# LepistaBioinformatics/blutils

Hardware: AMD Instinct MI355X
Metric: Mqueries/sec consensus (synthetic outfmt-6 hit table) (higher is better)
Workload: dtype i32/u32

## Files before the change

blutils_amd/csrc/consensus_kernel.hip:

```cpp

#if defined(__HIP_DEVICE_COMPILE__) && !defined(__gfx950__)
#error "consensus_kernel.hip is written for gfx950"
#endif

#include <hip/hip_runtime.h>

#include <climits>
#include <cstdint>
#include <type_traits>

#include "blu_internal.h"

namespace blu {

#define WAVE 64

constexpr int BLOCK_A = 768;
constexpr int BLU_WAVES_PER_SIMD = 3;
constexpr int BLOCK_N = 1024;
constexpr int BLU_N_WAVES_PER_SIMD = 4;
constexpr int BLOCK_F = 704;
constexpr int LIST_CAP = 208;
constexpr int LIST_CAP_RING = 248;
constexpr int LIST_CAP_F64 = 232;
// ... 263 lines not shown
#define KEY_PID_BITS 17u
#define KEYED_LEN_SHIFT 25u
#define KEYED_PID_SHIFT 8u
#define PM_MASK ((1u << KEY_PID_BITS) - 1u)
#define LONG_SPAN (1u << 28)
#define KEEP_ROWS 1024u
#define SLOT_CAP 256u
#define TASK_SPAN (1ull << 27)
#define CUT_LDS 512
#define ROW_MASK ((1u << BLU_ROW_BITS) - 1u)
typedef uint32_t u32x2 __attribute__((ext_vector_type(2)));
typedef uint32_t u32x4 __attribute__((ext_vector_type(4)));

static_assert((RING_ROWS & RING_MASK) == 0 && RING_ROWS >= 1024u, "ring size");
#define DESC_SUB_BITS 8u
#define DESC_WORD1(RPL, row0, sub) (((row0) << DESC_SUB_BITS) | (sub))
static_assert(LIST_CAP >= 128 && LIST_CAP_RING >= 128 && LIST_CAP_F64 >= 128 && LIST_CAP_F64_RING >= 128, "the list area also stages the 64 records of a task");
static_assert(LIST_CAP_RING % 8 == 0 && LIST_CAP_RING <= 256 && LIST_CAP_F64_RING % 8 == 0 && LIST_CAP_F64_RING <= 256, "four list entries per lane in the gather");

struct FlatLds { uint32_t qs[WAVE + 4]; int32_t qm[WAVE]; uint32_t qk[WAVE]; };
struct NoFlatLds {};
template <bool F64, bool RING>
struct WaveLds : std::conditional_t<RING, NoFlatLds, FlatLds> {
    static constexpr uint32_t CAP = F64 ? (RING ? LIST_CAP_F64_RING : LIST_CAP_F64) : (RING ? LIST_CAP_RING : LIST_CAP);
    alignas(16) uint32_t ring[RING ? RING_ROWS + RING_PAD : 4u];
    uint4 rec[CAP];
    uint32_t p1[F64 ? CAP : 1];
    uint16_t pq[CAP];
    uint32_t meta[WAVE + 4];
    uint2 seg[WAVE + 4];
};

__device__ __forceinline__ void wait_vmcnt(uint32_t k) {
    switch (k) {
        case 0: asm volatile("s_waitcnt vmcnt(0)" ::: "memory"); break;
        case 1: asm volatile("s_waitcnt vmcnt(1)" ::: "memory"); break;
        case 2: asm volatile("s_waitcnt vmcnt(2)" ::: "memory"); break;
        case 3: asm volatile("s_waitcnt vmcnt(3)" ::: "memory"); break;
        case 4: asm volatile("s_waitcnt vmcnt(4)" ::: "memory"); break;
        case 5: asm volatile("s_waitcnt vmcnt(5)" ::: "memory"); break;
        case 6: asm volatile("s_waitcnt vmcnt(6)" ::: "memory"); break;
        case 7: asm volatile("s_waitcnt vmcnt(7)" ::: "memory"); break;
        case 8: asm volatile("s_waitcnt vmcnt(8)" ::: "memory"); break;
        case 9: asm volatile("s_waitcnt vmcnt(9)" ::: "memory"); break;
        case 10: asm volatile("s_waitcnt vmcnt(10)" ::: "memory"); break;
        case 11: asm volatile("s_waitcnt vmcnt(11)" ::: "memory"); break;
        case 12: asm volatile("s_waitcnt vmcnt(12)" ::: "memory"); break;
        case 13: asm volatile("s_waitcnt vmcnt(13)" ::: "memory"); break;
        case 14: asm volatile("s_waitcnt vmcnt(14)" ::: "memory"); break;
        default: asm volatile("s_waitcnt vmcnt(15)" ::: "memory"); break;
    }
}
static_assert(RING_CHUNKS <= 16, "wait_vmcnt covers 0..15 younger chunks");

template <int STRAT, int LAYOUT, bool RING>
__global__ __launch_bounds__((LAYOUT == 0 || LAYOUT == 3) ? (RING ? BLOCK_F : BLOCK_A) : (RING ? BLOCK_A : BLOCK_N), (RING || LAYOUT == 0 || LAYOUT == 3) ? BLU_WAVES_PER_SIMD : BLU_N_WAVES_PER_SIMD)
void blu_consensus_stream_kernel(HitsDev h, TaxDev t, blu_result* __restrict__ out, uint32_t* __restrict__ worklist, uint32_t* __restrict__ work_count,
                                 uint32_t mode, uint32_t* __restrict__ host_len) {
    const uint32_t forced = mode & 1u;
    const bool no_long = (mode & 2u) != 0u;
    constexpr bool PID32 = LAYOUT == 1 || LAYOUT == 2, PACKED = LAYOUT == 2, WIDE = LAYOUT == 3;
    constexpr uint32_t BLOCK_T = !PID32 ? (RING ? BLOCK_F : BLOCK_A) : (RING ? BLOCK_A : BLOCK_N), WAVES_T = BLOCK_T / WAVE;
    constexpr uint32_t CAP = WaveLds<!PID32, RING>::CAP;
    if (!forced && __hip_atomic_load(work_count + 9, __ATOMIC_RELAXED, __HIP_MEMORY_SCOPE_AGENT) != (RING ? 1u : 2u)) return;
    __shared__ WaveLds<!PID32, RING> s_lds[WAVES_T];
    constexpr bool CUT_TABLE = !PID32;
    __shared__ double s_cut[CUT_TABLE ? CUT_LDS : 1];
    const bool cut_in_lds = CUT_TABLE && t.n_cutvals <= CUT_LDS;
    if constexpr (CUT_TABLE) {
        if (cut_in_lds) {
            for (uint32_t i = threadIdx.x; i < t.n_cutvals; i += BLOCK_T) s_cut[i] = t.cutvals[i];
            __syncthreads();
        }
    }
    int lane = lane_id();
    const int wib = __builtin_amdgcn_readfirstlane(threadIdx.x / WAVE);
    WaveLds<!PID32, RING>& L = s_lds[wib];
    const uint32_t wl_cap = wl_capacity(h.n_queries);
    const uint32_t n_q32 = (uint32_t)h.n_queries;
    const uint32_t wave = blockIdx.x * WAVES_T + (uint32_t)wib;
    const uint32_t n_waves = gridDim.x * WAVES_T;
    uint32_t t_full, tail_q0, tail_nq;
    {
        const uint32_t n_tasks64 = n_q32 / WAVE + ((n_q32 % WAVE) != 0u ? 1u : 0u);
        t_full = n_tasks64 / n_waves * n_waves;
        const uint32_t q_full = t_full == n_tasks64 ? n_q32 : t_full * WAVE;
        uint32_t tail_q = (((n_q32 - q_full) + n_waves - 1u) / n_waves + 7u) / 8u * 8u;
        tail_q = tail_q < 16u ? 16u : (tail_q > WAVE ? WAVE : tail_q);
        const uint64_t p0 = (uint64_t)q_full + (uint64_t)wave * tail_q;
        tail_q0 = p0 < n_q32 ? (uint32_t)p0 : n_q32;
        tail_nq = n_q32 - tail_q0 < tail_q ? n_q32 - tail_q0 : tail_q;
    }

    const uint32_t mis = (uint32_t)(((uintptr_t)h.bitscore >> 2) & 3u);
    const char* const bs_al = reinterpret_cast<const char*>(h.bitscore) - 4u * mis;
    const uint64_t v_total = h.n_hits + mis;
    uint32_t ring_head = 0, ring_landed = 0, ring_tail = 0;
    uint32_t ring_c0 = 0, ring_end = 0;
    uint32_t pref_q0 = 0xFFFFFFFFu;
    u32x4 rs_ring = {0u, 0u, 0u, 0x00020000u};
    auto ring_desc = [&](const uint32_t c0) {
        const uint64_t left = (v_total - ((uint64_t)c0 << 8)) * 4ull;
        const uint64_t base = (uint64_t)(uintptr_t)bs_al + ((uint64_t)c0 << 10);
        return u32x4{(uint32_t)__builtin_amdgcn_readfirstlane((int)(uint32_t)base),
                     (uint32_t)__builtin_amdgcn_readfirstlane((int)((uint32_t)(base >> 32) & 0xFFFFu)),
                     (uint32_t)__builtin_amdgcn_readfirstlane((int)(left < 0x80000000ull ? (uint32_t)left : 0x80000000u)), 0x00020000u};
// ... 1 lines not shown
    const uint32_t ring_lds = (uint32_t)__builtin_amdgcn_readfirstlane((int)(uint32_t)(uintptr_t)(__attribute__((address_space(3))) void*)L.ring);
    auto ring_dma_run = [&](const u32x4 rs, const uint32_t c0, uint32_t head, const uint32_t lim) {
        uint32_t voff = (head - c0) * 1024u + (uint32_t)lane * 16u, keep, t;
        asm volatile("s_mov_b32 %[keep], m0\n"
                     "1:\n\t"
                     "s_and_b32 %[t], %[head], %[cm]\n\t"
                     "s_lshl_b32 %[t], %[t], 10\n\t"
                     "s_add_u32 m0, %[t], %[base]\n\t"
                     "s_add_u32 %[head], %[head], 1\n\t"
                     "buffer_load_dwordx4 %[voff], %[rs], 0 offen" RING_DMA_MOD " lds\n\t"
                     "v_add_u32 %[voff], 0x400, %[voff]\n\t"
                     "s_cmp_lt_u32 %[head], %[lim]\n\t"
                     "s_cbranch_scc1 1b\n\t"
                     "s_mov_b32 m0, %[keep]"
                     : [keep] "=&s"(keep), [t] "=&s"(t), [head] "+s"(head), [voff] "+v"(voff)
                     : [cm] "n"(RING_CHUNKS - 1u), [base] "s"(ring_lds), [rs] "s"(rs), [lim] "s"(lim) : "memory", "scc");
    };

    const uint32_t n_hits32 = (uint32_t)h.n_hits;
    auto load_seg = [&](const uint32_t tq0, const uint32_t tnq, uint32_t& o, uint32_t& e) {
        o = 0; e = 0;
        if ((uint32_t)lane < tnq) {
            const uint32_t* lo32 = reinterpret_cast<const uint32_t*>(h.seg_off + ((uint64_t)tq0 + (uint32_t)lane));
            o = lo32[0]; e = lo32[2];
        }
    };
    uint32_t nx_off, nx_end;
    uint32_t task = wave;
    bool in_tail = task >= t_full, tail_done = false;
    load_seg(in_tail ? tail_q0 : task * WAVE, in_tail ? tail_nq : (uint32_t)WAVE, nx_off, nx_end);

    for (; !in_tail || (tail_nq != 0u && !tail_done); tail_done = in_tail, task += n_waves, in_tail = task >= t_full) {
        __builtin_amdgcn_s_setprio(0);
        asm volatile("" : "+v"(lane));
        const uint32_t q0_32 = in_tail ? tail_q0 : task * WAVE;
        const uint64_t q0 = q0_32;
        const uint32_t nq = in_tail ? tail_nq : (uint32_t)WAVE;
        const uint32_t wl_sel = (uint32_t)(q0 / WAVE) & (WL_QUEUES - 1u);
        uint32_t* const wl_cnt = work_count + WL_BASE + wl_sel * WL_STRIDE;
        uint32_t* const wl_q = worklist + (uint64_t)wl_sel * wl_cap;
        uint32_t my_off = nx_off, my_end = nx_end;
        if (my_end > n_hits32) my_end = n_hits32;
        if (my_off > my_end) my_off = my_end;
        const bool nx_tail = task + n_waves >= t_full;
        const uint32_t nx_q0 = nx_tail ? tail_q0 : (task + n_waves) * WAVE;
        const uint32_t nx_nq = in_tail ? 0u : (nx_tail ? tail_nq : (uint32_t)WAVE);
        load_seg(nx_q0, nx_nq, nx_off, nx_end);
        asm volatile("" ::: "memory");
        uint32_t fill = 0;
        bool keyed = false;
        bool keyed_bad = false;
        uint32_t scan_rpl = 16;
        uint32_t fill_ring = 0;
        const uint64_t q = q0 + (uint32_t)lane;
        const uint32_t row0 = my_off;
        uint32_t mode = 3, r_len = 0, r_row = 0, r_pos = 0, r_hdr = 0, minlen = 0, d = 0, rec_kind = 0, g_lo = 0, g_hi = 0;
        typedef typename PidKey<PID32>::type PK;
        PK r_pid = 0, max_pid = 0;
        uint4 ra = {0, 0, 0, 0}, rb = {0, 0, 0, 0};
        uint32_t st_code = 0, st_ref = 0;
        uint32_t dn_flag = 0, dn_err = 0, dn_pos = 0, dn_k = 0;
        bool in_span = true;
        const uint32_t task_start = (uint32_t)rl((int)my_off, 0);
        const uint64_t rem = (uint64_t)(n_hits32 - task_start) < TASK_SPAN ? (uint64_t)(n_hits32 - task_start) : TASK_SPAN;
        const uint32_t rem4 = (uint32_t)(rem * 4), rem8 = (uint32_t)(rem * 8);
        const auto rs_bs = __builtin_amdgcn_make_buffer_rsrc((void*)(h.bitscore + task_start), 0, rem4, 0x00020000);
        const auto rs_tax = PACKED ? __builtin_amdgcn_make_buffer_rsrc((void*)(h.packed + 4ull * task_start), 0, (uint32_t)(rem * 16), 0x00020000)
                            : WIDE ? __builtin_amdgcn_make_buffer_rsrc((void*)(h.packed64 + 6ull * task_start), 0, (uint32_t)(rem * 24), 0x00020000)
                                   : __builtin_amdgcn_make_buffer_rsrc((void*)(h.tax_row + task_start), 0, rem4, 0x00020000);
        const auto rs_aln = __builtin_amdgcn_make_buffer_rsrc((void*)(h.align_len + task_start), 0, rem4, 0x00020000);
        const auto rs_acc = __builtin_amdgcn_make_buffer_rsrc((void*)(h.acc_rank + task_start), 0, rem4, 0x00020000);
        const auto rs_pid = (PACKED || WIDE) ? rs_tax : PID32 ? __builtin_amdgcn_make_buffer_rsrc((void*)(h.pident_milli + task_start), 0, rem4, 0x00020000)
                                  : __builtin_amdgcn_make_buffer_rsrc((void*)(h.pident + task_start), 0, rem8, 0x00020000);
        {
            const uint32_t nrows = my_end - my_off;
            in_span = my_off >= task_start && (my_end - task_start) <= (uint32_t)TASK_SPAN;
            L.seg[lane] = make_uint2(my_off - task_start, (nrows <= MAX_TASK_SEG && in_span) ? nrows : 0u);
        }
        const uint32_t task_rows = ((uint32_t)lane < nq ? my_end : 0u) - ((uint32_t)lane < nq ? task_start : 0u);
        bool contiguous, all_short;
        {
            const uint32_t rel_end = my_end - task_start, rel_off = my_off - task_start;
            const uint32_t prev_end = (uint32_t)__shfl_up((int)rel_end, 1);
            const bool ok = in_span && (lane == 0 || rel_off == prev_end);
            contiguous = __ballot((uint32_t)lane < nq && !ok) == 0ull;
            all_short = __ballot((uint32_t)lane < nq && (my_end - my_off) > SHORT_SEG) == 0ull;
        }
        const uint32_t task_nrows = (uint32_t)rl((int)task_rows, (int)nq - 1);
        const uint64_t vbase = (uint64_t)task_start + mis;
        const uint32_t seg_x = my_off - task_start;
        struct StepRegs { u32x4 vbs, vtax, vp01, vp23, valn, vacc, vq; int left; uint32_t qi; };
        auto fetch_rest = [&](StepRegs& R, const uint32_t voff, const uint32_t rows) {
            const bool any = voff != 0xFFFFFFF0u && rows != 0u;
            if (PACKED) {
                const uint32_t base = voff * 4u;
                R.vtax = __builtin_amdgcn_raw_buffer_load_b128(rs_tax, (any && (rows & 1u)) ? base : 0xFFFFFFC0u, 0, STREAM_AUX);
                R.vp01 = __builtin_amdgcn_raw_buffer_load_b128(rs_tax, (any && (rows & 2u)) ? base + 16u : 0xFFFFFFC0u, 0, STREAM_AUX);
                R.valn = __builtin_amdgcn_raw_buffer_load_b128(rs_tax, (any && (rows & 4u)) ? base + 32u : 0xFFFFFFC0u, 0, STREAM_AUX);
                R.vacc = __builtin_amdgcn_raw_buffer_load_b128(rs_tax, (any && (rows & 8u)) ? base + 48u : 0xFFFFFFC0u, 0, STREAM_AUX);
                R.vp23 = R.vp01;
                return;
            }
            if (WIDE) {
                const uint32_t base = voff * 6u;
                R.vtax = __builtin_amdgcn_raw_buffer_load_b128(rs_tax, (any && (rows & 1u)) ? base : 0xFFFFFFC0u, 0, STREAM_AUX);
                R.vp01 = __builtin_amdgcn_raw_buffer_load_b128(rs_tax, (any && (rows & 2u)) ? base + 24u : 0xFFFFFFC0u, 0, STREAM_AUX);
// ... 329 lines not shown
                if (st >= ns) break;
                const uint32_t q = um[st] & 63u, oq = (um[st] >> 6) & 63u;
                const bool have = ((um[st] >> 12) & 15u) != 0u;
                const int M = L.qm[q];
                const uint32_t tmask = (have && lmx[st] == M) ? (um[st] >> 16) & 0xFFu : 0u;
                const uint32_t c = (uint32_t)__builtin_popcount(tmask);
                uint32_t in2 = c;
                in2 += (uint32_t)dpp<0x111>((int)in2);
                in2 += (uint32_t)dpp<0x112>((int)in2);
                in2 += (uint32_t)dpp<0x114>((int)in2);
                in2 += (uint32_t)dpp<0x118>((int)in2);
                const uint32_t k0 = (uint32_t)rl((int)in2, 15), k1 = (uint32_t)rl((int)in2, 31), k2 = (uint32_t)rl((int)in2, 47), k3 = (uint32_t)rl((int)in2, 63);
                in2 += r16 == 0 ? 0u : (r16 == 1 ? k0 : (r16 == 2 ? k0 + k1 : k0 + k1 + k2));
                const uint32_t idx0 = running + in2 - c;
                if (have && oq == 0u) L.meta[q] = META_SLOW | idx0;
                if (c) atomicAdd(&L.qk[q], c);
                const bool over = have && idx0 + c > CAP;
                const uint64_t over_m = __ballot(over);
                const bool room = !over && c != 0u && (over_m == 0ull || (uint32_t)lane < (uint32_t)__builtin_ctzll(over_m));
                if (room) L.rec[idx0] = make_uint4(__builtin_bitreverse32(tmask), L.seg[q].x + UR * oq, UR * oq, 0u);
                if (over_m) { q_cut = (uint32_t)rl((int)q, __builtin_ctzll(over_m)); break; }
                running += k0 + k1 + k2 + k3;
            }
            __builtin_amdgcn_fence(__ATOMIC_RELEASE, "workgroup");
            __builtin_amdgcn_wave_barrier();
            __builtin_amdgcn_fence(__ATOMIC_ACQUIRE, "workgroup");
            const uint32_t m = L.meta[lane];
            if (rows != 0u && (uint32_t)lane < q_cut) L.meta[lane] = (m & 0xFFFFu) | (L.qk[lane] << 16);
            fill = q_cut < q_lim ? (L.meta[q_cut] & 0xFFFFu) : running;
            if (q_cut < WAVE) stop_q = q_cut;
            }
        };
        auto ring_mark_landed = [&](const uint32_t upto) {
            const uint32_t m0 = (ring_landed + RING_CHUNKS - 1u) & ~(RING_CHUNKS - 1u);
            if (m0 < upto) {
                if ((uint32_t)lane < RING_PAD) L.ring[RING_ROWS + lane] = L.ring[lane];
                __builtin_amdgcn_fence(__ATOMIC_RELEASE, "workgroup");
                __builtin_amdgcn_wave_barrier();
                __builtin_amdgcn_fence(__ATOMIC_ACQUIRE, "workgroup");
            }
            ring_landed = upto;
        };
        auto ring_refill = [&]() {
            if (ring_head < ring_tail) { ring_head = ring_tail; if (ring_landed < ring_tail) ring_landed = ring_tail; }
            const uint32_t lim = ring_end < ring_tail + RING_CHUNKS ? ring_end : ring_tail + RING_CHUNKS;
            if (ring_head < lim) { ring_dma_run(rs_ring, ring_c0, ring_head, lim); ring_head = lim; }
        };
        auto phase1_scan = [&](const auto rpl_c, const auto full_c, const uint32_t LPQ) {
            constexpr uint32_t RPL = decltype(rpl_c)::value;
            constexpr bool FULL = decltype(full_c)::value;
            static_assert(RPL <= RING_PAD && RPL <= 32u, "rows per lane");
            const uint32_t QPS = WAVE / LPQ;
            const uint32_t grp = (uint32_t)lane / LPQ, sub = ((uint32_t)lane & (LPQ - 1u)) * RPL, row16 = (uint32_t)lane >> 4;
            {
                const uint32_t cs = (uint32_t)((vbase + (uint32_t)rl((int)seg_x, (int)first_q)) >> 8);
                if (cs < ring_tail) { wait_vmcnt(0u); ring_head = ring_landed = ring_tail = cs; }
            }
            for (uint32_t qb = first_q / QPS * QPS; qb < nq; qb += QPS) {
                const uint32_t r_lo = (uint32_t)rl((int)seg_x, (int)(qb < first_q ? first_q : qb));
                const uint32_t qn = qb + QPS;
                const uint32_t r_hi = qn < nq ? (uint32_t)rl((int)seg_x, (int)qn) : task_nrows;
                ring_tail = (uint32_t)((vbase + r_lo) >> 8);
                ring_refill();
                if (r_hi > r_lo) {
                    const uint32_t need = (uint32_t)((vbase + r_hi - 1u) >> 8);
                    if (need >= ring_landed) { wait_vmcnt(ring_head - 1u - need); ring_mark_landed(need + 1u); }
                }
                const uint32_t qi = qb + grp;
                const uint2 sg = L.seg[qi];
                const int left0 = (sg.y > short_seg ? 0 : (int)sg.y) - (int)sub;
                const uint32_t over = (FULL && left0 > 0 && left0 < (int)RPL) ? RPL - (uint32_t)left0 : 0u;
                const uint32_t sub_e = sub - over;
                const int left = FULL ? (left0 > 0 ? (int)RPL : 0) : left0;
                const uint32_t row0 = sg.x + sub_e;
                const uint32_t a = ((uint32_t)vbase + sg.x + sub_e) & RING_MASK;
                int b[RPL];
#pragma unroll
                for (uint32_t i = 0; i < RPL; ++i) b[i] = (int)L.ring[a + i];
                asm volatile("s_waitcnt lgkmcnt(0)" ::: "memory");
#pragma unroll
                for (uint32_t i = 0; i < RPL; ++i) asm volatile("" : "+v"(b[i]));
                if (r_hi > r_lo) { ring_tail = (uint32_t)((vbase + r_hi) >> 8); ring_refill(); }
                int M = INT_MIN;
                if constexpr (FULL) {
#pragma unroll
                    for (uint32_t i = 0; i < RPL; ++i) M = imax(M, b[i]);
                    M = left > 0 ? M : INT_MIN;
                } else {
#pragma unroll
                    for (uint32_t i = 0; i < RPL; ++i) { b[i] = (int)i < left ? b[i] : INT_MIN; M = imax(M, b[i]); }
                }
                if (LPQ >= 2) M = imax(M, dpp<0xB1>(M));
                if (LPQ >= 4) M = imax(M, dpp<0x4E>(M));
                if (LPQ >= 8) M = imax(M, dpp<0x141>(M));
                if (LPQ >= 16) M = imax(M, dpp<0x140>(M));
                uint32_t mask = tie_mask<RPL>(b, M);
                mask = left > 0 ? mask : 0u;
                if constexpr (FULL) mask &= 0xFFFFFFFFu >> (32u - RPL + over);
                const uint32_t c = (uint32_t)__builtin_popcount(mask);
                uint32_t incl = c;
                incl += (uint32_t)dpp<0x111>((int)incl);
                incl += (uint32_t)dpp<0x112>((int)incl);
                incl += (uint32_t)dpp<0x114>((int)incl);
                incl += (uint32_t)dpp<0x118>((int)incl);
                const uint32_t k0 = (uint32_t)rl((int)incl, 15), k1 = (uint32_t)rl((int)incl, 31);
                const uint32_t k2 = (uint32_t)rl((int)incl, 47), k3 = (uint32_t)rl((int)incl, 63);
                const bool fits = fill + k0 + k1 + k2 + k3 <= CAP;
                const uint32_t p1 = fill + k0, p2 = p1 + k1, p3 = p2 + k2;
                const uint32_t rbase = row16 == 0 ? fill : (row16 == 1 ? p1 : (row16 == 2 ? p2 : p3));
                uint32_t gk = c;
                if (LPQ >= 2) gk += (uint32_t)dpp<0xB1>((int)gk);
                if (LPQ >= 4) gk += (uint32_t)dpp<0x4E>((int)gk);
                if (LPQ >= 8) gk += (uint32_t)dpp<0x141>((int)gk);
                if (LPQ >= 16) gk += (uint32_t)dpp<0x140>((int)gk);
                if (PID32 && !fits) {
                    __builtin_amdgcn_s_setprio(2);
                    uint64_t BK = 0;
                    uint32_t bacc = 0, bpos = 0, brow = 0, kmin = 0xFFFFFFFFu, pmax = 0, dlo = 0xFFFFFFFFu, dhi = 0, err = 0xFFFFFFFFu;
                    auto reset = [&]() { BK = 0; bacc = 0; bpos = 0; brow = 0; kmin = 0xFFFFFFFFu; pmax = 0; dlo = 0xFFFFFFFFu; dhi = 0; err = 0xFFFFFFFFu; };
                    auto better = [&](const uint64_t K, const uint32_t acc, const uint32_t pos, const uint64_t K2, const uint32_t acc2, const uint32_t pos2) {
                        const bool gt = (K > K2) | ((K == K2) & (acc > acc2)), eq = (K == K2) & (acc == acc2);
                        return STRAT == BLU_RELAXED ? (gt | (eq & (pos > pos2))) : ((!gt & !eq) | (eq & (pos < pos2)));
                    };
                    auto take_record = [&](const u32x4 rec, const uint32_t gp, const bool on) {
                        const uint32_t len = umin(rec.x >> BLU_ROW_BITS, t.max_depth), pos = rec.x & ROW_MASK;
                        const bool unmatched = pos >= t.n_tax, bad = !unmatched && (rec.x >> BLU_ROW_BITS) == 0;
                        const uint32_t e = (gp << 8) | (bad ? (uint32_t)BLU_ST_ERR_BAD_LINEAGE : (uint32_t)BLU_ST_ERR_UNMATCHED_TAXID);
                        err = (on && (unmatched | bad)) ? umin(err, e) : err;
                        const uint32_t pm = rec.y & ((1u << KEY_PID_BITS) - 1u);
                        const uint32_t k1 = (len << KEY_PID_BITS) | pm;
                        const uint64_t K = ((uint64_t)k1 << 32) | (rec.z ^ 0x80000000u);
                        const bool take = on & ((kmin == 0xFFFFFFFFu) | better(K, rec.w, gp, BK, bacc, bpos));
                        BK = take ? K : BK; bacc = take ? rec.w : bacc; bpos = take ? gp : bpos; brow = take ? pos : brow;
                        kmin = on ? umin(kmin, k1) : kmin;
                        const uint32_t pmo = pm | ((!PACKED && rec.y >= (1u << KEY_PID_BITS)) ? 0x80000000u : 0u);
                        pmax = (on && pmo > pmax) ? pmo : pmax;
                        dlo = on ? umin(dlo, pos) : dlo;
                        dhi = (on && pos > dhi) ? pos : dhi;
                    };
                    auto load_record = [&](const uint32_t row, const bool on) {
                        u32x4 r;
                        if (PACKED) r = __builtin_amdgcn_raw_buffer_load_b128(rs_tax, on ? row * 16u : 0xFFFFFFC0u, 0, GATHER_AUX);
                        else {
                            const uint32_t o4 = on ? row * 4u : 0xFFFFFFF0u;
                            r.x = __builtin_amdgcn_raw_buffer_load_b32(rs_tax, o4, 0, GATHER_AUX);
                            r.y = __builtin_amdgcn_raw_buffer_load_b32(rs_pid, o4, 0, GATHER_AUX);
                            r.z = __builtin_amdgcn_raw_buffer_load_b32(rs_aln, o4, 0, GATHER_AUX);
                            r.w = __builtin_amdgcn_raw_buffer_load_b32(rs_acc, o4, 0, GATHER_AUX);
                        }
                        return r;
                    };
                    auto merge = [&](auto ctrl) {
                        constexpr int C = decltype(ctrl)::value;
                        const uint64_t K2 = ((uint64_t)(uint32_t)dpp<C>((int)(uint32_t)(BK >> 32)) << 32) | (uint32_t)dpp<C>((int)(uint32_t)BK);
                        const uint32_t acc2 = (uint32_t)dpp<C>((int)bacc), pos2 = (uint32_t)dpp<C>((int)bpos), row2 = (uint32_t)dpp<C>((int)brow);
                        const uint32_t kmin2 = (uint32_t)dpp<C>((int)kmin);
                        const bool take = (kmin2 != 0xFFFFFFFFu) & ((kmin == 0xFFFFFFFFu) | better(K2, acc2, pos2, BK, bacc, bpos));
                        BK = take ? K2 : BK; bacc = take ? acc2 : bacc; bpos = take ? pos2 : bpos; brow = take ? row2 : brow;
                        kmin = umin(kmin, kmin2);
                        const uint32_t pm2 = (uint32_t)dpp<C>((int)pmax); pmax = pm2 > pmax ? pm2 : pmax;
                        dlo = umin(dlo, (uint32_t)dpp<C>((int)dlo));
                        const uint32_t hi2 = (uint32_t)dpp<C>((int)dhi); dhi = hi2 > dhi ? hi2 : dhi;
                        err = umin(err, (uint32_t)dpp<C>((int)err));
                    };
                    auto deliver = [&](const int src, const bool mine) {
                        const uint32_t f_khi = (uint32_t)__builtin_amdgcn_ds_bpermute(src, (int)(uint32_t)(BK >> 32));
                        const uint32_t f_pos = (uint32_t)__builtin_amdgcn_ds_bpermute(src, (int)bpos), f_row = (uint32_t)__builtin_amdgcn_ds_bpermute(src, (int)brow);
// ... 43 lines not shown
                            if (LPQ >= 2) merge(std::integral_constant<int, 0x141>());
                            if (LPQ >= 4) merge(std::integral_constant<int, 0x140>());
                            deliver((int)(((own0 & 15u) * 4u) * 4u), mine && (own0 >> 4) == g);
                        }
                    } else {
                        uint32_t m = mask;
                        while (__ballot(m != 0u)) {
                            u32x4 rq[4];
                            uint32_t gp[4];
#pragma unroll
                            for (int j = 0; j < 4; ++j) {
                                const bool on = m != 0u;
                                const uint32_t hb = on ? 31u - (uint32_t)__builtin_clz(m) : 0u, i = RPL - 1u - hb;
                                m = on ? (m & ~(1u << hb)) : 0u;
                                gp[j] = on ? sub_e + i : 0xFFFFFFFFu;
                                rq[j] = load_record(row0 + i, on);
                            }
#pragma unroll
                            for (int j = 0; j < 4; ++j) take_record(rq[j], gp[j], gp[j] != 0xFFFFFFFFu);
                        }
                        if (LPQ >= 2) merge(std::integral_constant<int, 0xB1>());
                        if (LPQ >= 4) merge(std::integral_constant<int, 0x4E>());
                        if (LPQ >= 8) merge(std::integral_constant<int, 0x141>());
                        if (LPQ >= 16) merge(std::integral_constant<int, 0x140>());
                        deliver((int)(own0 * 4u), mine);
                    }
                    {
                        const uint32_t f_gk = (uint32_t)__builtin_amdgcn_ds_bpermute((int)(own0 * 4u), (int)gk);
                        dn_k = (mine && dn_flag == 1u) ? f_gk : dn_k;
                    }
                    if (sub == 0 && gk != 0u) L.meta[qi] = META_DENSE;
                    __builtin_amdgcn_s_setprio(0);
                    continue;
                }
                uint32_t idx = rbase + incl - c;
                if (!fits) {
                    const uint32_t lane_o = (uint32_t)__builtin_ctzll(__ballot(idx + c > CAP));
                    const uint32_t qo = qb + lane_o / LPQ;
                    const bool taken = qi < qo;
                    if (sub == 0) L.meta[qi] = taken ? (idx | (gk << 16)) : META_SLOW;
                    if (taken && c) { L.rec[idx].x = mask << (32u - RPL); L.rec[idx].y = DESC_WORD1(RPL, row0, sub_e); }
                    fill = (uint32_t)rl((int)idx, (int)((qo - qb) * LPQ));
                    stop_q = qo;
                    wait_vmcnt(0u);
                    ring_head = ring_landed = ring_tail = (uint32_t)((vbase + (uint32_t)rl((int)seg_x, (int)qo)) >> 8);
                    break;
                }
                if (sub == 0) L.meta[qi] = idx | (gk << 16);
                fill = p3 + k3;
                static_assert((RPL == 16u || RPL == 32u) && SHORT_SEG <= 128u, "descriptor word of a lane");
                if (c) { L.rec[idx].x = mask << (32u - RPL); L.rec[idx].y = DESC_WORD1(RPL, row0, sub_e); }
            }
        };
        auto gather_list = [&](auto&& between) {
            constexpr int NG = (CAP + WAVE - 1) / WAVE;
            u32x4 g[NG];
            uint32_t ghi[NG], gpos[NG], ghint[NG];
            uint32_t carry = 0;
#pragma unroll
            for (int u = 0; u < NG; ++u) {
                g[u] = u32x4{0u, 0u, 0u, 0u}; ghi[u] = 0u; gpos[u] = 0u; ghint[u] = 0u;
                if ((uint32_t)u * WAVE >= fill_ring) continue;
                const uint32_t idx = (uint32_t)u * WAVE + (uint32_t)lane;
                const bool valid = idx < fill_ring;
                const uint32_t d0 = L.rec[idx < CAP ? idx : 0u].x;
                int s = (valid && d0 != 0u) ? (int)idx : 0;
                s = imax(s, dpp<0x111>(s));
                s = imax(s, dpp<0x112>(s));
                s = imax(s, dpp<0x114>(s));
                s = imax(s, dpp<0x118>(s));
                s = imax(s, __builtin_amdgcn_update_dpp(0, s, 0x142, 0xA, 0xF, false));
                s = imax(s, __builtin_amdgcn_update_dpp(0, s, 0x143, 0xC, 0xF, false));
                s = imax(s, (int)carry);
                carry = (uint32_t)rl(s, 63);
                const uint4 dd = L.rec[s];
                const uint32_t d0w = dd.x, d = dd.y;
                uint32_t r = idx - (uint32_t)s, x = scan_rpl == 32u ? d0w : d0w >> 16, i = 0;
                if (scan_rpl == 32u) {
                    const uint32_t h = x >> 16, ch = (uint32_t)__builtin_popcount(h);
                    const bool low = r >= ch;
                    r -= low ? ch : 0u; x = low ? (x & 0xFFFFu) : h; i += low ? 16u : 0u;
                }
                {
                    const uint32_t h = x >> 8, ch = (uint32_t)__builtin_popcount(h);
                    const bool low = r >= ch;
                    r -= low ? ch : 0u; x = low ? (x & 0xFFu) : h; i += low ? 8u : 0u;
                }
                {
                    const uint32_t h = x >> 4, ch = (uint32_t)__builtin_popcount(h);
                    const bool low = r >= ch;
                    r -= low ? ch : 0u; x = low ? (x & 0xFu) : h; i += low ? 4u : 0u;
                }
                {
                    const uint32_t h = x >> 2, ch = (uint32_t)__builtin_popcount(h);
                    const bool low = r >= ch;
                    r -= low ? ch : 0u; x = low ? (x & 0x3u) : h; i += low ? 2u : 0u;
                }
                i += (r >= (x >> 1)) ? 1u : 0u;
                const uint32_t row = (RING ? (d >> DESC_SUB_BITS) : d) + i;
                gpos[u] = (RING ? (d & ((1u << DESC_SUB_BITS) - 1u)) : dd.z) + i;
                if (PACKED) g[u] = __builtin_amdgcn_raw_buffer_load_b128(rs_tax, valid ? row * 16u : 0xFFFFFFC0u, 0, GATHER_AUX);
                else if (WIDE) {
                    g[u] = __builtin_amdgcn_raw_buffer_load_b128(rs_tax, valid ? row * 24u : 0xFFFFFFC0u, 0, GATHER_AUX);
                    const u32x2 p = __builtin_amdgcn_raw_buffer_load_b64(rs_tax, valid ? row * 24u + 16u : 0xFFFFFFE0u, 0, GATHER_AUX);
                    ghint[u] = g[u].y;
                    g[u].y = p.x; ghi[u] = p.y;
                } else {
                    const uint32_t o4 = valid ? row * 4u : 0xFFFFFFF0u;
                    g[u].x = __builtin_amdgcn_raw_buffer_load_b32(rs_tax, o4, 0, GATHER_AUX);
                    if (PID32) g[u].y = __builtin_amdgcn_raw_buffer_load_b32(rs_pid, o4, 0, GATHER_AUX);
                    else {
                        const u32x2 p = __builtin_amdgcn_raw_buffer_load_b64(rs_pid, valid ? row * 8u : 0xFFFFFFE0u, 0, GATHER_AUX);
                        g[u].y = p.x; ghi[u] = p.y;
                    }
                    g[u].z = __builtin_amdgcn_raw_buffer_load_b32(rs_aln, o4, 0, GATHER_AUX);
                    g[u].w = __builtin_amdgcn_raw_buffer_load_b32(rs_acc, o4, 0, GATHER_AUX);
                }
            }
            between();
            bool ovf = false;
            uint32_t gk[NG];
#pragma unroll
            for (int u = 0; u < NG; ++u) {
                const bool valid = (uint32_t)u * WAVE + (uint32_t)lane < fill_ring;
                if constexpr (PID32) { gk[u] = g[u].y & PM_MASK; ovf |= !PACKED && valid && g[u].y >= (1u << KEY_PID_BITS); }
                else {
                    const double p = __hiloint2double((int)ghi[u], (int)g[u].y);
                    const bool in_range = p >= 0.0 && p < 131.0705;
                    const uint32_t k = in_range ? (uint32_t)(p * 1000.0 + 0.5) : 0u;
                    const double back = milli17_to_f64(k);
                    gk[u] = k;
                    ovf |= valid && !(in_range && __double2hiint(back) == (int)ghi[u] && __double2loint(back) == (int)g[u].y && k < BLU_KTHR_NEVER);
                }
            }
            keyed = __ballot(ovf) == 0ull && fill == fill_ring;
            bool any_bad = false;
#pragma unroll
            for (int u = 0; u < NG; ++u) {
                const uint32_t idx = (uint32_t)u * WAVE + (uint32_t)lane;
                if (idx < fill_ring) {
                    if (keyed) {
                        const uint32_t len = umin(g[u].x >> BLU_ROW_BITS, t.max_depth);
                        any_bad |= len == 0u || (g[u].x & ROW_MASK) >= t.n_tax;
                        const uint32_t hint = (PID32 ? g[u].y : ghint[u]) >> KEY_PID_BITS;
                        L.rec[idx] = make_uint4((g[u].x & ROW_MASK) | ((hint >> 8) << BLU_ROW_BITS),
                                                (len << KEYED_LEN_SHIFT) | (gk[u] << KEYED_PID_SHIFT) | (hint & 0xFFu), g[u].z ^ 0x80000000u, g[u].w);
                    } else L.rec[idx] = make_uint4(g[u].x, g[u].y, g[u].z, g[u].w);
                    L.pq[idx] = (uint16_t)gpos[u];
                    if (!PID32) L.p1[idx] = ghi[u];
                }
            }
            keyed_bad = __ballot(any_bad) != 0ull;
        };
        bool pend = (uint32_t)lane < nq;
        uint32_t pend_before = WAVE + 1;
        if (RING && contiguous) {
            ring_c0 = (uint32_t)(vbase >> 8);
            rs_ring = ring_desc(ring_c0);
            ring_end = task_nrows ? (uint32_t)((vbase + task_nrows - 1u) >> 8) + 1u : ring_c0;
            if (pref_q0 != q0_32) ring_head = ring_landed = ring_c0;
            ring_tail = ring_c0;
        }
        for (;;) {
        fill = 0;
        stop_q = WAVE;
        bool ring_round = false;
        bool list_round = false;
        keyed = false;
        {
            const uint32_t rows = L.seg[lane].y;
            const uint64_t live = __ballot(rows != 0u);
            first_q = live ? (uint32_t)__builtin_ctzll(live) : 0u;
            {
                const uint32_t n16 = (uint32_t)__builtin_popcountll(__ballot(rows != 0u && rows <= 16u));
                const uint32_t n32 = (uint32_t)__builtin_popcountll(__ballot(rows != 0u && rows <= 32u));
                const uint32_t n64 = (uint32_t)__builtin_popcountll(__ballot(rows != 0u && rows <= 64u));
                const uint32_t n128 = (uint32_t)__builtin_popcountll(__ballot(rows != 0u && rows <= SHORT_SEG));
                const uint32_t c16 = 4u * n16 + BLU_LONG_COST * (n128 - n16), c32 = 8u * n32 + BLU_LONG_COST * (n128 - n32);
                const uint32_t c64 = 16u * n64 + BLU_LONG_COST * (n128 - n64), c128 = 32u * n128;
                uint32_t best = c128;
                short_seg = SHORT_SEG;
                if (c64 < best) { best = c64; short_seg = 64u; }
                if (c32 < best) { best = c32; short_seg = 32u; }
                if (c16 < best) { best = c16; short_seg = 16u; }
            }
            bool flat_round = false;
            if constexpr (!RING) {
                const uint32_t n128 = (uint32_t)__builtin_popcountll(__ballot(rows != 0u && rows <= SHORT_SEG));
                const uint32_t n_over = (uint32_t)__builtin_popcountll(__ballot(rows > SHORT_SEG));
                uint32_t best;
                {
                    const uint32_t n16 = (uint32_t)__builtin_popcountll(__ballot(rows != 0u && rows <= 16u));
                    const uint32_t n32 = (uint32_t)__builtin_popcountll(__ballot(rows != 0u && rows <= 32u));
                    const uint32_t n64 = (uint32_t)__builtin_popcountll(__ballot(rows != 0u && rows <= 64u));
                    best = 32u * n128;
                    best = umin(best, 16u * n64 + BLU_LONG_COST * (n128 - n64));
                    best = umin(best, 8u * n32 + BLU_LONG_COST * (n128 - n32));
                    best = umin(best, 4u * n16 + BLU_LONG_COST * (n128 - n16));
                }
                const uint32_t units = (uint32_t)wave_sum_u32((rows + FLAT_ROWS - 1u) / FLAT_ROWS);
                flat_round = units != 0u && units + units / 4u + 64u < best + BLU_LONG_COST * n_over;
                if (flat_round) { short_seg = FLAT_SEG; scan_rpl = 16u; }
            }
            const uint32_t longest = flat_round ? 0u : wave_max_u32(rows > short_seg ? 0u : rows);
            ring_round = RING && contiguous && longest != 0u && all_short && __ballot(rows > short_seg) == 0ull;
            uint32_t lpq = 1;
            if (ring_round) {
                scan_rpl = longest > 32u ? 32u : 16u;
                while (lpq * scan_rpl < longest) lpq *= 2;
                while ((WAVE / lpq) * longest + 256u > RING_ROWS) lpq *= 2;
            }
            list_round = ring_round || flat_round;
            if (list_round) {
#pragma unroll
                for (uint32_t u = 0; u * WAVE < CAP; ++u) { const uint32_t i = u * WAVE + (uint32_t)lane; if (i < CAP) L.rec[i].x = 0u; }
            }
            if (ring_round) {
                const bool all_full = __ballot(rows != 0u && rows <= short_seg && rows < scan_rpl) == 0ull;
                if (scan_rpl == 32u) {
                    if (all_full) phase1_scan(std::integral_constant<uint32_t, 32>(), std::true_type(), lpq);
                    else phase1_scan(std::integral_constant<uint32_t, 32>(), std::false_type(), lpq);
                } else phase1_scan(std::integral_constant<uint32_t, 16>(), std::false_type(), lpq);
            }
            else if (flat_round) phase1_flat();
            else if (longest > 32u && longest <= 64u) phase1(std::integral_constant<uint32_t, 16>(), false);
            else if (longest) phase1(longest <= 16u ? 4u : (longest <= 32u ? 8u : 32u), longest >= (PACKED ? 9u : 25u));
            if (stop_q < WAVE && rows != 0u && ((uint32_t)lane >= stop_q || rows > short_seg)) L.meta[lane] = META_SLOW;
            fill_ring = list_round ? fill : 0u;
            const uint64_t long_mask = __ballot(rows > short_seg);
            if (long_mask && stop_q == WAVE) phase1_long(long_mask);
        }
        __builtin_amdgcn_fence(__ATOMIC_RELEASE, "workgroup");
        __builtin_amdgcn_wave_barrier();
        __builtin_amdgcn_fence(__ATOMIC_ACQUIRE, "workgroup");
        const bool last_round = __ballot(pend && (my_end - my_off) != 0u && (my_end - my_off) <= MAX_TASK_SEG && in_span && (L.meta[lane] & META_SLOW)) == 0ull;
        uint32_t nxt_c0 = 0, nxt_lim = 0;
        if (RING && last_round && nx_nq != 0u) {
            uint32_t n_off = nx_off, n_end = nx_end;
            asm volatile("" : "+v"(n_off), "+v"(n_end));
            if (n_end > n_hits32) n_end = n_hits32;
            if (n_off > n_end) n_off = n_end;
            const uint32_t nqn = nx_nq;
            const uint32_t n_start = (uint32_t)rl((int)n_off, 0);
            const bool n_span = n_off >= n_start && (n_end - n_start) <= (uint32_t)TASK_SPAN;
            const uint32_t rel_end = n_end - n_start, rel_off = n_off - n_start;
            const uint32_t prev_end = (uint32_t)__shfl_up((int)rel_end, 1);
            const bool ok = n_span && (n_end - n_off) <= SHORT_SEG && (lane == 0 || rel_off == prev_end);
            const uint32_t n_rows = (uint32_t)rl((int)rel_end, (int)nqn - 1);
            if (__ballot((uint32_t)lane < nqn && !ok) == 0ull && n_rows != 0u) {
                const uint64_t vb = (uint64_t)n_start + mis;
                nxt_c0 = (uint32_t)(vb >> 8);
                const uint32_t cend = (uint32_t)((vb + n_rows - 1u) >> 8) + 1u;
                nxt_lim = cend < nxt_c0 + RING_CHUNKS ? cend : nxt_c0 + RING_CHUNKS;
            }
        }
        auto prefetch_next = [&]() {
            if (nxt_lim > nxt_c0) {
                const auto rsn = ring_desc(nxt_c0);
                ring_dma_run(rsn, nxt_c0, nxt_c0, nxt_lim);
                ring_head = nxt_lim; ring_landed = nxt_c0; ring_tail = nxt_c0;
                pref_q0 = nx_q0;
            }
        };
        __builtin_amdgcn_s_setprio(3);
        if (list_round) gather_list(prefetch_next);
        else prefetch_next();
        __builtin_amdgcn_fence(__ATOMIC_RELEASE, "workgroup");
        __builtin_amdgcn_wave_barrier();
        __builtin_amdgcn_fence(__ATOMIC_ACQUIRE, "workgroup");

        {
            const uint32_t nrows = my_end - my_off;
            const uint32_t m = L.meta[lane];
            const bool listed = pend && nrows != 0 && nrows <= MAX_TASK_SEG && in_span && !(m & (META_SLOW | META_DENSE));
            const uint32_t first = listed ? (m & 0xFFFFu) : 0u, k = listed ? ((m >> 16) & 0x3FFu) : 0u;
            const uint32_t kmax = wave_max_u32(k);
            uint32_t err = 0, err_pos = 0, nan_pos = 0xFFFFFFFFu;
            uint32_t b_len = 0, b_acc = 0, lo = 0xFFFFFFFFu, hi = 0, l_minlen = 0xFFFFFFFFu, l_row = 0, l_pos = 0, l_hint = 0;
            int b_aln = 0;
            PK b_pid = 0, l_maxpid = 0;
            const uint32_t last_e = k ? k - 1u : 0u;
            uint4 nx_rec = make_uint4(0, 0, 0, 0);
            uint32_t nx_pq = 0;
            uint32_t l_keyed = 0;
            if (!keyed) { nx_rec = L.rec[first]; nx_pq = L.pq[first]; }
            if (keyed) {
                l_keyed = 1u;
                uint64_t BK = 0;
                uint32_t kmin = 0xFFFFFFFFu, pmax = 0;
                uint32_t l_idx = first;
                auto step = [&](const auto check_c, const uint4 x, const uint32_t xidx, const bool is_first) {
                    const uint32_t pos = x.x & ROW_MASK;
                    if constexpr (decltype(check_c)::value) {
                        const bool unmatched = pos >= t.n_tax, bad = x.y < (1u << KEYED_LEN_SHIFT);
                        const bool first_err = (err == 0) & (unmatched | bad);
                        err = first_err ? (unmatched ? (uint32_t)BLU_ST_ERR_UNMATCHED_TAXID : (uint32_t)BLU_ST_ERR_BAD_LINEAGE) : err;
                        err_pos = first_err ? (uint32_t)L.pq[xidx] : err_pos;
                    }
                    kmin = umin(kmin, x.y);
                    lo = umin(lo, pos);
                    hi = pos > hi ? pos : hi;
                    const uint32_t ky = x.y & ~0xFFu;
                    const uint32_t pm = (x.y >> KEYED_PID_SHIFT) & PM_MASK;
                    pmax = pm > pmax ? pm : pmax;
                    const uint64_t K = ((uint64_t)ky << 32) | x.z;
                    const bool gt = (K > BK) | ((K == BK) & (x.w > b_acc)), eq = (K == BK) & (x.w == b_acc);
                    const bool take = is_first | (STRAT == BLU_RELAXED ? (gt | eq) : !(gt | eq));
                    BK = take ? K : BK;
                    b_acc = take ? x.w : b_acc;
                    l_idx = take ? xidx : l_idx;
                };
                auto reduce = [&](const auto check_c) {
                    for (uint32_t e = 0; e < kmax; e += 4) {
                        uint4 x[4];
                        uint32_t xi[4];
// ... 728 lines not shown
```

Before: 11400.

## Gather packed taxonomy rows via direct-to-LDS DMA and defer overflowing scan groups

For the packed ring layout, the list gather now issues buffer_load ... lds instructions that write the gathered 16-byte taxonomy records straight into LDS behind the ring. The wait is counted, so the next task's ring prefetch can stay in flight while the gather completes, and the results are then re-keyed in place. When a scan group would overflow the list, the scan stops early, saves that group's descriptor, and resumes it in a later round instead of taking the slow fallback path. This avoids register staging and the full vmcnt drain, at the cost of inline asm with manual m0 juggling and more complex round state.

```diff
diff --git a/blutils_amd/csrc/consensus_kernel.hip b/blutils_amd/csrc/consensus_kernel.hip
--- a/blutils_amd/csrc/consensus_kernel.hip
+++ b/blutils_amd/csrc/consensus_kernel.hip
@@ -339,6 +339,9 @@
     }
 }
 static_assert(RING_CHUNKS <= 16, "wait_vmcnt covers 0..15 younger chunks");
+constexpr uint32_t GATHER_REQS = (LIST_CAP_RING + WAVE - 1) / WAVE;
+static_assert(RING_CHUNKS + GATHER_REQS <= 15u, "ring chunks and gather requests in flight together fit the counted wait");
+__device__ __forceinline__ void gather_wait(const uint32_t chunks_behind) { wait_vmcnt(chunks_behind); }
 
 template <int STRAT, int LAYOUT, bool RING>
 __global__ __launch_bounds__((LAYOUT == 0 || LAYOUT == 3) ? (RING ? BLOCK_F : BLOCK_A) : (RING ? BLOCK_A : BLOCK_N), (RING || LAYOUT == 0 || LAYOUT == 3) ? BLU_WAVES_PER_SIMD : BLU_N_WAVES_PER_SIMD)
@@ -446,6 +449,8 @@
         bool keyed_bad = false;
         uint32_t scan_rpl = 16;
         uint32_t fill_ring = 0;
+        uint32_t dz_mask = 0, dz_w1 = 0, dz_qb = 0, dz_lpq = 0, scan_from = 0xFFFFFFFFu;
+        bool dz_on = false;
         const uint64_t q = q0 + (uint32_t)lane;
         const uint32_t row0 = my_off;
         uint32_t mode = 3, r_len = 0, r_row = 0, r_pos = 0, r_hdr = 0, minlen = 0, d = 0, rec_kind = 0, g_lo = 0, g_hi = 0;
@@ -881,11 +886,12 @@
             static_assert(RPL <= RING_PAD && RPL <= 32u, "rows per lane");
             const uint32_t QPS = WAVE / LPQ;
             const uint32_t grp = (uint32_t)lane / LPQ, sub = ((uint32_t)lane & (LPQ - 1u)) * RPL, row16 = (uint32_t)lane >> 4;
-            {
+            const bool resume = PACKED && scan_from != 0xFFFFFFFFu;
+            if (!resume) {
                 const uint32_t cs = (uint32_t)((vbase + (uint32_t)rl((int)seg_x, (int)first_q)) >> 8);
                 if (cs < ring_tail) { wait_vmcnt(0u); ring_head = ring_landed = ring_tail = cs; }
             }
-            for (uint32_t qb = first_q / QPS * QPS; qb < nq; qb += QPS) {
+            for (uint32_t qb = resume ? scan_from : first_q / QPS * QPS; qb < nq; qb += QPS) {
                 const uint32_t r_lo = (uint32_t)rl((int)seg_x, (int)(qb < first_q ? first_q : qb));
                 const uint32_t qn = qb + QPS;
                 const uint32_t r_hi = qn < nq ? (uint32_t)rl((int)seg_x, (int)qn) : task_nrows;
@@ -942,6 +948,11 @@
                 if (LPQ >= 4) gk += (uint32_t)dpp<0x4E>((int)gk);
                 if (LPQ >= 8) gk += (uint32_t)dpp<0x141>((int)gk);
                 if (LPQ >= 16) gk += (uint32_t)dpp<0x140>((int)gk);
+                if (PACKED && !fits && fill != 0u && k0 + k1 + k2 + k3 <= CAP) {
+                    dz_mask = mask << (32u - RPL); dz_w1 = DESC_WORD1(RPL, row0, sub_e); dz_qb = qb; dz_lpq = LPQ; dz_on = true;
+                    stop_q = qb;
+                    break;
+                }
                 if (PID32 && !fits) {
                     __builtin_amdgcn_s_setprio(2);
                     uint64_t BK = 0;
@@ -1091,8 +1102,104 @@
                 if (c) { L.rec[idx].x = mask << (32u - RPL); L.rec[idx].y = DESC_WORD1(RPL, row0, sub_e); }
             }
         };
+        auto entry_of = [&](const uint32_t idx, const bool valid, uint32_t& carry, uint32_t& row, uint32_t& pos) {
+            const uint32_t d0 = L.rec[idx < CAP ? idx : 0u].x;
+            int s = (valid && d0 != 0u) ? (int)idx : 0;
+            s = imax(s, dpp<0x111>(s));
+            s = imax(s, dpp<0x112>(s));
+            s = imax(s, dpp<0x114>(s));
+            s = imax(s, dpp<0x118>(s));
+            s = imax(s, __builtin_amdgcn_update_dpp(0, s, 0x142, 0xA, 0xF, false));
+            s = imax(s, __builtin_amdgcn_update_dpp(0, s, 0x143, 0xC, 0xF, false));
+            s = imax(s, (int)carry);
+            carry = (uint32_t)rl(s, 63);
+            const uint4 dd = L.rec[s];
+            const uint32_t d0w = dd.x, d = dd.y;
+            uint32_t r = idx - (uint32_t)s, x = scan_rpl == 32u ? d0w : d0w >> 16, i = 0;
+            if (scan_rpl == 32u) {
+                const uint32_t h = x >> 16, ch = (uint32_t)__builtin_popcount(h);
+                const bool low = r >= ch;
+                r -= low ? ch : 0u; x = low ? (x & 0xFFFFu) : h; i += low ? 16u : 0u;
+            }
+            {
+                const uint32_t h = x >> 8, ch = (uint32_t)__builtin_popcount(h);
+                const bool low = r >= ch;
+                r -= low ? ch : 0u; x = low ? (x & 0xFFu) : h; i += low ? 8u : 0u;
+            }
+            {
+                const uint32_t h = x >> 4, ch = (uint32_t)__builtin_popcount(h);
+                const bool low = r >= ch;
+                r -= low ? ch : 0u; x = low ? (x & 0xFu) : h; i += low ? 4u : 0u;
+            }
+            {
+                const uint32_t h = x >> 2, ch = (uint32_t)__builtin_popcount(h);
+                const bool low = r >= ch;
+                r -= low ? ch : 0u; x = low ? (x & 0x3u) : h; i += low ? 2u : 0u;
+            }
+            i += (r >= (x >> 1)) ? 1u : 0u;
+            row = (RING ? (d >> DESC_SUB_BITS) : d) + i;
+            pos = (RING ? (d & ((1u << DESC_SUB_BITS) - 1u)) : dd.z) + i;
+        };
         auto gather_list = [&](auto&& between) {
             constexpr int NG = (CAP + WAVE - 1) / WAVE;
+            if constexpr (PACKED && RING) {
+                static_assert(sizeof(L.ring) % 16u == 0u && NG * WAVE * 16u <= 0x10000u, "the list starts right behind the ring; DMA destinations are 16-byte aligned");
+                uint32_t grow[NG], gp[NG];
+                uint32_t carry = 0;
+#pragma unroll
+                for (int u = 0; u < NG; ++u) {
+                    grow[u] = 0u; gp[u] = 0u;
+                    if ((uint32_t)u * WAVE >= fill_ring) continue;
+                    const uint32_t idx = (uint32_t)u * WAVE + (uint32_t)lane;
+                    const bool valid = idx < fill_ring;
+                    uint32_t row, pos;
+                    entry_of(idx, valid, carry, row, pos);
+                    grow[u] = row * 16u;
+                    gp[u] = pos;
+                }
+                asm volatile("s_waitcnt lgkmcnt(0)" ::: "memory");
+                const uint64_t gbase = (uint64_t)(uintptr_t)(h.packed + 4ull * task_start);
+                const u32x4 rs_g = {(uint32_t)__builtin_amdgcn_readfirstlane((int)(uint32_t)gbase),
+                                    (uint32_t)__builtin_amdgcn_readfirstlane((int)((uint32_t)(gbase >> 32) & 0xFFFFu)),
+                                    (uint32_t)__builtin_amdgcn_readfirstlane((int)(uint32_t)(rem * 16)), 0x00020000u};
+#pragma unroll
+                for (int u = 0; u < NG; ++u) {
+                    if ((uint32_t)u * WAVE >= fill_ring) continue;
+                    const uint32_t idx = (uint32_t)u * WAVE + (uint32_t)lane;
+                    if (idx < fill_ring) {
+                        L.pq[idx] = (uint16_t)gp[u];
+                        uint32_t keep;
+                        asm volatile("s_mov_b32 %[keep], m0\n\t"
+                                     "s_add_u32 m0, %[base], %[off]\n\t"
+                                     "s_nop 4\n\t"
+                                     "buffer_load_dwordx4 %[voff], %[rs], 0 offen nt lds\n\t"
+                                     "s_mov_b32 m0, %[keep]"
+                                     : [keep] "=&s"(keep)
+                                     : [base] "s"(ring_lds), [off] "n"((uint32_t)sizeof(L.ring) + (uint32_t)u * WAVE * 16u), [voff] "v"(grow[u]), [rs] "s"(rs_g)
+                                     : "memory", "scc");
+                    }
+                }
+                const uint32_t behind = between();
+                gather_wait(behind);
+                keyed = fill == fill_ring;
+                bool any_bad = false;
+                if (keyed) {
+#pragma unroll
+                    for (int u = 0; u < NG; ++u) {
+                        const uint32_t idx = (uint32_t)u * WAVE + (uint32_t)lane;
+                        if (idx < fill_ring) {
+                            const uint4 g = L.rec[idx];
+                            const uint32_t len = umin(g.x >> BLU_ROW_BITS, t.max_depth);
+                            any_bad |= len == 0u || (g.x & ROW_MASK) >= t.n_tax;
+                            const uint32_t hint = g.y >> KEY_PID_BITS;
+                            L.rec[idx] = make_uint4((g.x & ROW_MASK) | ((hint >> 8) << BLU_ROW_BITS),
+                                                    (len << KEYED_LEN_SHIFT) | ((g.y & PM_MASK) << KEYED_PID_SHIFT) | (hint & 0xFFu), g.z ^ 0x80000000u, g.w);
+                        }
+                    }
+                }
+                keyed_bad = __ballot(any_bad) != 0ull;
+                return;
+            }
             u32x4 g[NG];
             uint32_t ghi[NG], gpos[NG], ghint[NG];
             uint32_t carry = 0;
@@ -1102,42 +1209,8 @@
                 if ((uint32_t)u * WAVE >= fill_ring) continue;
                 const uint32_t idx = (uint32_t)u * WAVE + (uint32_t)lane;
                 const bool valid = idx < fill_ring;
-                const uint32_t d0 = L.rec[idx < CAP ? idx : 0u].x;
-                int s = (valid && d0 != 0u) ? (int)idx : 0;
-                s = imax(s, dpp<0x111>(s));
-                s = imax(s, dpp<0x112>(s));
-                s = imax(s, dpp<0x114>(s));
-                s = imax(s, dpp<0x118>(s));
-                s = imax(s, __builtin_amdgcn_update_dpp(0, s, 0x142, 0xA, 0xF, false));
-                s = imax(s, __builtin_amdgcn_update_dpp(0, s, 0x143, 0xC, 0xF, false));
-                s = imax(s, (int)carry);
-                carry = (uint32_t)rl(s, 63);
-                const uint4 dd = L.rec[s];
-                const uint32_t d0w = dd.x, d = dd.y;
-                uint32_t r = idx - (uint32_t)s, x = scan_rpl == 32u ? d0w : d0w >> 16, i = 0;
-                if (scan_rpl == 32u) {
-                    const uint32_t h = x >> 16, ch = (uint32_t)__builtin_popcount(h);
-                    const bool low = r >= ch;
-                    r -= low ? ch : 0u; x = low ? (x & 0xFFFFu) : h; i += low ? 16u : 0u;
-                }
-                {
-                    const uint32_t h = x >> 8, ch = (uint32_t)__builtin_popcount(h);
-                    const bool low = r >= ch;
-                    r -= low ? ch : 0u; x = low ? (x & 0xFFu) : h; i += low ? 8u : 0u;
-                }
-                {
-                    const uint32_t h = x >> 4, ch = (uint32_t)__builtin_popcount(h);
-                    const bool low = r >= ch;
-                    r -= low ? ch : 0u; x = low ? (x & 0xFu) : h; i += low ? 4u : 0u;
-                }
-                {
-                    const uint32_t h = x >> 2, ch = (uint32_t)__builtin_popcount(h);
-                    const bool low = r >= ch;
-                    r -= low ? ch : 0u; x = low ? (x & 0x3u) : h; i += low ? 2u : 0u;
-                }
-                i += (r >= (x >> 1)) ? 1u : 0u;
-                const uint32_t row = (RING ? (d >> DESC_SUB_BITS) : d) + i;
-                gpos[u] = (RING ? (d & ((1u << DESC_SUB_BITS) - 1u)) : dd.z) + i;
+                uint32_t row;
+                entry_of(idx, valid, carry, row, gpos[u]);
                 if (PACKED) g[u] = __builtin_amdgcn_raw_buffer_load_b128(rs_tax, valid ? row * 16u : 0xFFFFFFC0u, 0, GATHER_AUX);
                 else if (WIDE) {
                     g[u] = __builtin_amdgcn_raw_buffer_load_b128(rs_tax, valid ? row * 24u : 0xFFFFFFC0u, 0, GATHER_AUX);
@@ -1242,9 +1315,11 @@
                 if (flat_round) { short_seg = FLAT_SEG; scan_rpl = 16u; }
             }
             const uint32_t longest = flat_round ? 0u : wave_max_u32(rows > short_seg ? 0u : rows);
-            ring_round = RING && contiguous && longest != 0u && all_short && __ballot(rows > short_seg) == 0ull;
+            const bool waiting = PACKED && RING && dz_on;
+            ring_round = waiting || (RING && contiguous && longest != 0u && all_short && __ballot(rows > short_seg) == 0ull);
             uint32_t lpq = 1;
-            if (ring_round) {
+            if (waiting) { lpq = dz_lpq; short_seg = SHORT_SEG; }
+            else if (ring_round) {
                 scan_rpl = longest > 32u ? 32u : 16u;
                 while (lpq * scan_rpl < longest) lpq *= 2;
                 while ((WAVE / lpq) * longest + 256u > RING_ROWS) lpq *= 2;
@@ -1253,6 +1328,28 @@
             if (list_round) {
 #pragma unroll
                 for (uint32_t u = 0; u * WAVE < CAP; ++u) { const uint32_t i = u * WAVE + (uint32_t)lane; if (i < CAP) L.rec[i].x = 0u; }
+            }
+            scan_from = 0xFFFFFFFFu;
+            if (waiting) {
+                const uint32_t c = (uint32_t)__builtin_popcount(dz_mask), row16 = (uint32_t)lane >> 4;
+                uint32_t incl = c;
+                incl += (uint32_t)dpp<0x111>((int)incl);
+                incl += (uint32_t)dpp<0x112>((int)incl);
+                incl += (uint32_t)dpp<0x114>((int)incl);
+                incl += (uint32_t)dpp<0x118>((int)incl);
+                const uint32_t k0 = (uint32_t)rl((int)incl, 15), k1 = (uint32_t)rl((int)incl, 31);
+                const uint32_t k2 = (uint32_t)rl((int)incl, 47), k3 = (uint32_t)rl((int)incl, 63);
+                const uint32_t idx = (row16 == 0 ? 0u : (row16 == 1 ? k0 : (row16 == 2 ? k0 + k1 : k0 + k1 + k2))) + incl - c;
+                uint32_t gk = c;
+                if (lpq >= 2) gk += (uint32_t)dpp<0xB1>((int)gk);
+                if (lpq >= 4) gk += (uint32_t)dpp<0x4E>((int)gk);
+                if (lpq >= 8) gk += (uint32_t)dpp<0x141>((int)gk);
+                if (lpq >= 16) gk += (uint32_t)dpp<0x140>((int)gk);
+                if (((uint32_t)lane & (lpq - 1u)) == 0u) L.meta[dz_qb + (uint32_t)lane / lpq] = idx | (gk << 16);
+                if (c) { L.rec[idx].x = dz_mask; L.rec[idx].y = dz_w1; }
+                fill = k0 + k1 + k2 + k3;
+                scan_from = dz_qb + WAVE / lpq;
+                dz_on = false;
             }
             if (ring_round) {
                 const bool all_full = __ballot(rows != 0u && rows <= short_seg && rows < scan_rpl) == 0ull;
@@ -1293,13 +1390,15 @@
                 nxt_lim = cend < nxt_c0 + RING_CHUNKS ? cend : nxt_c0 + RING_CHUNKS;
             }
         }
-        auto prefetch_next = [&]() {
+        auto prefetch_next = [&]() -> uint32_t {
             if (nxt_lim > nxt_c0) {
                 const auto rsn = ring_desc(nxt_c0);
                 ring_dma_run(rsn, nxt_c0, nxt_c0, nxt_lim);
                 ring_head = nxt_lim; ring_landed = nxt_c0; ring_tail = nxt_c0;
                 pref_q0 = nx_q0;
-            }
+                return nxt_lim - nxt_c0;
+            }
+            return 0u;
         };
         __builtin_amdgcn_s_setprio(3);
         if (list_round) gather_list(prefetch_next);
```

After: 10850. 0.952x the previous value.
